# Zhongxu-Wang/ArtSpeech

Measured on AMD Instinct MI355X. Metric: mel frames/sec (whole job; per-GPU = value / n_gpus), acoustic-model inference path, batch 32 x 200-frame utterances, higher is better.
Workload: dtype f32 (f16x3 split-operand MFMA, fp32 accumulate)

## Files before the change

artspeech_amd/csrc/conv_gemm_h3.hip:

```cpp
#include "conv_gemm.h"
#include <cstring>
#include <type_traits>

typedef __attribute__((address_space(3))) void lds_void;

template <int I, int N, typename F>
static __device__ __forceinline__ void h3_for(F&& f)
{
    if constexpr (I < N) {
        f(std::integral_constant<int, I>{});
        h3_for<I + 1, N>(f);
    }
}

template <int WM, int WN, int WK, int KT, int NS, int NP, int TM = 2>
struct H3Cfg {
    static constexpr int QP = NP == 1 ? 2 : 4;
    static constexpr int BM = 32 * TM * WM, BN = 64 * WN;
    static constexpr int KBS = WK * KT;
    static constexpr int A_BLK = QP * BM * 16, B_BLK = QP * BN * 16;
    static constexpr int A_ST = KBS * A_BLK;
    static constexpr int STAGE = KBS * (A_BLK + B_BLK);
    static constexpr int RED = (WK - 1) * WM * WN * 32 * TM * 64 * 4;
    static constexpr int LDS = NS * STAGE > RED ? NS * STAGE : RED;
    static constexpr int NT = 64 * WM * WN * WK;
    static constexpr int ACH = KBS * QP * BM / NT;
    static constexpr int BCH = KBS * QP * BN / NT;
    static constexpr int NMF = 2 * TM * NP;
    static constexpr int NFR = (TM + 2) * (NP == 1 ? 1 : 2);
};

static constexpr int H3_OCC = 1;
static __device__ __forceinline__ int h3_problem_of(const H3Multi& mm)
{
    int pi = 0;
#pragma unroll
    for (int i = 1; i < H3_MAXP; ++i) pi += (i < mm.n && (int)blockIdx.x >= mm.p[i].wg0) ? 1 : 0;
    return pi;
}

template <int WM, int WN, int WK, int KT, int NS, int NP, int TM = 2>
static __device__ __forceinline__ void h3_tile(const H3Prob& prob, unsigned char* smem)
{
    using C = H3Cfg<WM, WN, WK, KT, NS, NP, TM>;
    static_assert(NS >= 2 && NS <= 4, "stages");
    constexpr int BM = C::BM, BN = C::BN, ACH = C::ACH, BCH = C::BCH, NT = C::NT, QP = C::QP, KBS = C::KBS;
    static_assert(NT == 256 && ACH * NT == KBS * QP * BM && BCH * NT == KBS * QP * BN && ACH >= 1 && BCH >= 1, "tile shape");

    const int tid = threadIdx.x, lane = tid & 63;
    const int wave = __builtin_amdgcn_readfirstlane(tid >> 6);
    const int wk = wave / (WM * WN), wmn = wave % (WM * WN), wm = wmn % WM, wn = wmn / WM;
    const int l31 = lane & 31, lk = lane >> 5;
    const ConvGemmArgs& a = prob.a;
    const H3Taps& tp = prob.tp;
    const int S = prob.S;
    const int tiles_m = (a.M + BM - 1) / BM;
    int lt, slice, tile, m0, n0, grp = 0, n_end = prob.col1;
    if (a.n_valid && S == 1) {
        const int nv = __builtin_amdgcn_readfirstlane(*a.n_valid);
        const int G = a.n_groups > 1 ? a.n_groups : 1;
        const int span = G > 1 ? a.group_cols : prob.col1 - prob.col0;
        const int ctv = (min(max(nv, 1), span) + BN - 1) / BN;
        const int tiles_v = tiles_m * G * ctv, per = (tiles_v + 7) >> 3;
        const int local = (int)blockIdx.x - prob.wg0;
        if ((local >> 3) >= per) return;
        lt = (local & 7) * per + (local >> 3);
        if (lt >= tiles_v) return;
        slice = 0;
        tile = lt;
        m0 = (lt % tiles_m) * BM;
        const int q = lt / tiles_m, tn = q / G;
        grp = q - tn * G;
        const int base = G > 1 ? grp * a.group_cols : prob.col0;
        n0 = base + tn * BN;
        n_end = min(G > 1 ? min(a.N, (grp + 1) * a.group_cols) : prob.col1, base + nv);
    } else {
        lt = logical_of((int)blockIdx.x - prob.wg0, prob.wgs);
        if (lt >= prob.tiles * S) return;
        slice = lt / prob.tiles;
        tile = lt - slice * prob.tiles;
        m0 = (tile % tiles_m) * BM;
        n0 = prob.col0 + (tile / tiles_m) * BN;
        if (a.n_groups > 1) {
            const int tpg = (a.group_cols + BN - 1) / BN, tn = tile / tiles_m;
            grp = tn / tpg;
            n0 = grp * a.group_cols + (tn - grp * tpg) * BN;
            n_end = min(a.N, (grp + 1) * a.group_cols);
        }
        if (a.n_valid) {
            n_end = min(n_end, (a.n_groups > 1 ? grp * a.group_cols : 0) + __builtin_amdgcn_readfirstlane(*a.n_valid));
            if (n0 >= n_end && n0 > 0) return;
        }
    }
    const int KB = a.Kp >> 4, KBx = (KB + 3) & ~3;
    const int NX = (a.src_col ? a.N_in : a.N) + 1;

    const int KB2 = (a.K2 + 15) >> 4, KBx2 = (KB2 + 3) & ~3;
    const unsigned w_bytes = ((unsigned)a.T * KBx + KBx2) * 4u * a.M * 16u;
    const __amdgpu_buffer_rsrc_t rsW = __builtin_amdgcn_make_buffer_rsrc(
        const_cast<unsigned char*>(reinterpret_cast<const unsigned char*>(a.Wh) + (size_t)grp * w_bytes), 0, (int)w_bytes, 0x00020000);
    const __amdgpu_buffer_rsrc_t rsX = __builtin_amdgcn_make_buffer_rsrc(
        const_cast<uint16_t*>(a.Xh), 0, (int)((unsigned)KBx * 4u * NX * 16u), 0x00020000);
    const __amdgpu_buffer_rsrc_t rsX2 = __builtin_amdgcn_make_buffer_rsrc(
        const_cast<uint16_t*>(KB2 ? a.Xh2 : a.Xh), 0, (int)((unsigned)KBx2 * 4u * NX * 16u), 0x00020000);

    (void)rsW;
    (void)rsX;
    (void)rsX2;
    unsigned a_voff[ACH];
#pragma unroll
    for (int i = 0; i < ACH; ++i) {
        const int c = tid + NT * i, kblk = c / (QP * BM), rem = c % (QP * BM), pk = rem / BM, row = rem % BM;
        a_voff[i] = (m0 + row) < a.M ? (unsigned)(((kblk * 4 + pk) * a.M + m0 + row) * 16) : OOB;
    }
    unsigned b_plane[BCH];
#pragma unroll
    for (int i = 0; i < BCH; ++i) {
        const int c = tid + NT * i, kblk = c / (QP * BN), pk = (c % (QP * BN)) / BN;
        b_plane[i] = (unsigned)((kblk * 4 + pk) * NX) * 16u;
    }
    const int j = n0 + tid % BN;
    unsigned tapmask = 0;
    int Wj = 0;
    if (j < n_end) {
        if (a.meta) {
            const unsigned long long md = a.meta[j];
            const int h = AS_META_h(md), w = AS_META_w(md);
            const int H = AS_META_H(md);
            Wj = AS_META_W(md);
            for (int t = 0; t < a.T; ++t) {
                const int byte = (int)(h3_tap_word(tp, t) >> ((t & 7) * 8)) & 0xff;
                const int dh = tp.wide ? 0 : (byte >> 4) - 8, dw = tp.wide ? byte - 128 : (byte & 15) - 8;
                if ((unsigned)(h + dh) < (unsigned)H && (unsigned)(w + dw) < (unsigned)Wj) tapmask |= 1u << t;
            }
        } else {
            tapmask = 0xffffffffu;
        }
    }
    const int jsrc = a.src_col ? (j < n_end ? a.src_col[j] : 0) : j;
    const int tA = tp.wide ? 16 : Wj, tC = jsrc + (tp.wide ? -128 : -8 * Wj - 8);

    const int it_per_tap = (KB + KBS - 1) / KBS;
    const int nit_all = a.T * it_per_tap + (KB2 + KBS - 1) / KBS;
    const int it_lo = (int)((long)nit_all * slice / S);
    const int n_it = (int)((long)nit_all * (slice + 1) / S) - it_lo;

    int s_t = min(it_lo / it_per_tap, a.T), s_kb = (it_lo - s_t * it_per_tap) * KBS;
    int kb_lim = s_t < a.T ? KB : KB2;
    __amdgpu_buffer_rsrc_t rsXc = s_t < a.T ? rsX : rsX2;
    const int a_step = KBS * 4 * a.M * 16, b_step = KBS * 4 * NX * 16;
    int a_soff = (s_t * KBx + s_kb) * 4 * a.M * 16, b_soff = s_kb * 4 * NX * 16;
    unsigned bv[BCH];
    auto set_tap = [&](int t) {
        int byte = (int)(h3_tap_word(tp, t) >> ((t & 7) * 8)) & 0xff;
        unsigned ok = 0u - ((tapmask >> (t & 31)) & 1u);
        if (t >= a.T) {
            byte = tp.wide ? 128 : 0x88;
            ok = 0u - (unsigned)(j < n_end);
        }
        const unsigned src = ((unsigned)((byte >> 4) * tA + (byte & 15) + tC) & ok) | ((unsigned)(NX - 1) & ~ok);
#pragma unroll
        for (int i = 0; i < BCH; ++i) bv[i] = b_plane[i] + src * 16u;
    };
    set_tap(s_t);
    auto advance = [&]() {
        s_kb += KBS;
        a_soff += a_step;
        b_soff += b_step;
        if (s_kb >= kb_lim) {
            if (s_t + 1 < a.T || (s_t + 1 == a.T && KB2 > 0)) {
                s_t += 1;
                s_kb = 0;
                a_soff = s_t * KBx * 4 * a.M * 16;
                b_soff = 0;
                if (s_t == a.T) {
                    kb_lim = KB2;
                    rsXc = rsX2;
                }
                set_tap(s_t);
            } else {
                s_kb -= KBS;
                a_soff -= a_step;
                b_soff -= b_step;
            }
        }
    };
    auto dma_a = [&](auto i_, int stage) {
#if __HIP_DEVICE_COMPILE__
        constexpr int i = decltype(i_)::value;
        __builtin_amdgcn_raw_ptr_buffer_load_lds(rsW, (lds_void*)(smem + stage * C::STAGE + wave * 1024 + i * (NT * 16)), 16, a_voff[i],
                                                 a_soff, 0, 0);
#endif
    };
    auto dma_b = [&](auto i_, int stage) {
#if __HIP_DEVICE_COMPILE__
        constexpr int i = decltype(i_)::value;
        __builtin_amdgcn_raw_ptr_buffer_load_lds(rsXc, (lds_void*)(smem + stage * C::STAGE + C::A_ST + wave * 1024 + i * (NT * 16)), 16, bv[i],
                                                 b_soff, 0, 0);
#endif
    };
    (void)bv;
    (void)a_soff;
    (void)b_soff;
    (void)rsXc;
    f16x8 fa[2][TM][2], fb[2][2][2];
    const int a_frag = (wk * KT * QP + lk) * BM * 16 + (wm * 32 * TM + l31) * 16;
    const int b_frag = C::A_ST + (wk * KT * QP + lk) * BN * 16 + (wn * 64 + l31) * 16;
    auto read_frag = [&](auto q_, auto set_, auto s_, int stage) {
        constexpr int q = decltype(q_)::value, set = decltype(set_)::value, s = decltype(s_)::value;
        constexpr int sec = q < TM ? 0 : (q < TM + 2 ? 1 : (q < 2 * TM + 2 ? 2 : 3));
        constexpr int i = sec == 0 ? q : (sec == 1 ? q - TM : (sec == 2 ? q - TM - 2 : q - 2 * TM - 2));
        constexpr int ab = sec == 0 || sec == 2 ? 0 : 1;
        constexpr int p = NP == 1 ? 0 : (sec == 0 || sec == 3 ? 0 : 1);
        const unsigned char* st = smem + stage * C::STAGE;
        if constexpr (ab == 0) fa[set][i][p] = *reinterpret_cast<const f16x8*>(st + a_frag + (s * QP + p * 2) * BM * 16 + i * 32 * 16);
        else fb[set][i][p] = *reinterpret_cast<const f16x8*>(st + b_frag + (s * QP + p * 2) * BN * 16 + i * 32 * 16);
    };
    f32x16 acc[TM][2];
#pragma unroll
    for (int i = 0; i < TM; ++i)
#pragma unroll
        for (int jn = 0; jn < 2; ++jn)
#pragma unroll
            for (int e = 0; e < 16; ++e) acc[i][jn][e] = 0.f;

    using I0 = std::integral_constant<int, 0>;
    constexpr int L = KT == 1 ? NS : NS - 1;
    static_assert(L >= 2, "KT > 1 needs three stages");
    for (int st = 0; st < L; ++st) {
        h3_for<0, ACH>([&](auto i_) { dma_a(i_, st); });
        h3_for<0, BCH>([&](auto i_) { dma_b(i_, st); });
        advance();
    }
    __syncthreads();
    h3_for<0, C::NFR>([&](auto q_) { read_frag(q_, I0{}, I0{}, 0); });
    __syncthreads();

    constexpr int NMI = KT * C::NMF;
    constexpr int M_ADV = ACH + BCH, NMS = M_ADV + 1;
    constexpr int SLOT0 = 0;
    auto stage_micro = [&](auto m_, auto p_) {
        constexpr int Mi = decltype(m_)::value, P = (decltype(p_)::value + L) % NS;
        if constexpr (Mi < ACH) dma_a(std::integral_constant<int, Mi>{}, P);
        else if constexpr (Mi < M_ADV) dma_b(std::integral_constant<int, Mi - ACH>{}, P);
        else advance();
    };
    auto slot_of_stage = [](int m) constexpr { return SLOT0 + (m * (NMI - SLOT0)) / NMS; };
    auto slot_of_frag = [](int s, int q) constexpr {
        return s * C::NMF + (q * (C::NMF - 2)) / C::NFR + (C::NMF > 4 ? 1 : 0);
    };
    auto step = [&](auto n_, auto s_, auto p_, auto f_) {
        constexpr int Nn = decltype(n_)::value, Ss = decltype(s_)::value, P = decltype(p_)::value, F = decltype(f_)::value;
        constexpr int grp_ = Nn / (2 * TM), i = (Nn % (2 * TM)) / 2, jn = Nn % 2;
        constexpr int PA = NP == 1 ? 0 : (grp_ == 1 ? 1 : 0);
        constexpr int PB = NP == 1 ? 0 : (grp_ == 0 ? 1 : 0);
        acc[i][jn] = __builtin_amdgcn_mfma_f32_32x32x16_f16(fa[F][i][PA], fb[F][jn][PB], acc[i][jn], 0, 0, 0);
        constexpr int slot = Ss * C::NMF + Nn;
        h3_for<0, NMS>([&](auto m_) {
            if constexpr (slot_of_stage(decltype(m_)::value) == slot) stage_micro(m_, p_);
        });
        h3_for<0, C::NFR>([&](auto q_) {
            if constexpr (slot_of_frag(Ss, decltype(q_)::value) == slot) {
                if constexpr (Ss + 1 < KT) read_frag(q_, std::integral_constant<int, F ^ 1>{}, std::integral_constant<int, Ss + 1>{}, P);
                else read_frag(q_, std::integral_constant<int, F ^ 1>{}, I0{}, (P + 1) % NS);
            }
        });
        __builtin_amdgcn_sched_barrier(0);
    };
    constexpr int PEND = (L - 2) * (ACH + BCH);
#define H3_ITER(U)                                                                                                \
    {                                                                                                             \
        h3_for<0, KT>([&](auto s_) {                                                                              \
            h3_for<0, C::NMF>([&](auto n_) {                                                                      \
                step(n_, s_, std::integral_constant<int, (U) % NS>{},                                             \
                     std::integral_constant<int, ((U) * KT + decltype(s_)::value) % 2>{});                        \
            });                                                                                                   \
        });                                                                                                       \
        asm volatile("s_waitcnt vmcnt(%0) lgkmcnt(0)\n\ts_barrier" ::"n"(PEND) : "memory");                     \
    }
    constexpr int PERIOD = (KT % 2 == 0) ? NS : (NS % 2 == 0 ? NS : 2 * NS);
    int it = 0;
    for (; it + PERIOD <= n_it; it += PERIOD) {
        h3_for<0, PERIOD>([&](auto u_) { H3_ITER(decltype(u_)::value) });
    }
    h3_for<0, PERIOD - 1>([&](auto u_) {
        if (it + decltype(u_)::value < n_it) H3_ITER(decltype(u_)::value)
    });
#undef H3_ITER
    asm volatile("s_waitcnt vmcnt(0)\n\ts_barrier" ::: "memory");

    if (WK > 1) {
        f32x4* red = reinterpret_cast<f32x4*>(smem);
        if (wk > 0) {
#pragma unroll
            for (int i = 0; i < TM; ++i)
#pragma unroll
                for (int jn = 0; jn < 2; ++jn)
#pragma unroll
                    for (int e4 = 0; e4 < 4; ++e4) {
                        f32x4 v = {acc[i][jn][4 * e4], acc[i][jn][4 * e4 + 1], acc[i][jn][4 * e4 + 2], acc[i][jn][4 * e4 + 3]};
                        red[((((wk - 1) * (WM * WN) + wmn) * 2 * TM + i * 2 + jn) * 4 + e4) * 64 + lane] = v;
                    }
        }
        __syncthreads();
        if (wk == 0)
#pragma unroll
            for (int s = 1; s < WK; ++s)
#pragma unroll
                for (int i = 0; i < TM; ++i)
#pragma unroll
                    for (int jn = 0; jn < 2; ++jn)
#pragma unroll
                        for (int e4 = 0; e4 < 4; ++e4) {
                            const f32x4 v = red[((((s - 1) * (WM * WN) + wmn) * 2 * TM + i * 2 + jn) * 4 + e4) * 64 + lane];
#pragma unroll
                            for (int c = 0; c < 4; ++c) acc[i][jn][4 * e4 + c] += v[c];
                        }
    }
    epilogue<TM, 2>(a, acc, m0, n0, wm, wn, l31, lk, S, slice, wk == 0, grp, n_end);
}

template <int WM, int WN, int WK, int KT, int NS, int NP, int TM = 2>
__global__ void __launch_bounds__(64 * WM * WN * WK, H3_OCC)
conv_gemm_h3_kernel(const H3Multi mm)
{
    extern __shared__ __attribute__((aligned(16))) unsigned char smem[];
    h3_tile<WM, WN, WK, KT, NS, NP, TM>(mm.p[h3_problem_of(mm)], smem);
}

template <int WM, int WN, int WK, int KT, int NS, int NP, int TM = 2>
static int launch_h3(const ConvGemmArgs* const* a, const int* S, int n, hipStream_t stream)
{
    using C = H3Cfg<WM, WN, WK, KT, NS, NP, TM>;
    AS_LDS_OPT_IN((&conv_gemm_h3_kernel<WM, WN, WK, KT, NS, NP, TM>), C::LDS);
    H3Multi mm;
    memset(&mm, 0, sizeof(mm));
    mm.n = n;
    int wg = 0;
    for (int i = 0; i < n; ++i) {
        H3Prob& p = mm.p[i];
        p.a = *a[i];
        if (h3_pack_taps(p.a, &p.tp) != AS_OK) return AS_EINVAL;
        const int tiles_n = p.a.n_groups > 1 ? p.a.n_groups * as_cdiv(p.a.group_cols, C::BN) : as_cdiv(p.a.N, C::BN);
        p.tiles = as_cdiv(p.a.M, C::BM) * tiles_n;
        p.col0 = 0;
        p.col1 = p.a.N;
        p.S = S[i];
        p.wg0 = wg;
        p.wgs = (p.tiles * p.S + 7) & ~7;
        wg += p.wgs;
    }
    hipLaunchKernelGGL((conv_gemm_h3_kernel<WM, WN, WK, KT, NS, NP, TM>), dim3(wg), dim3(C::NT), C::LDS, stream, mm);
    AS_CHECK_LAUNCH();
    return AS_OK;
}

template <int WM, int WN, int WK>
static int launch_h3_tile(const ConvGemmArgs* const* a, const int* S, int n, hipStream_t stream)
{
    if (a[0]->n_prod == 1) return launch_h3<WM, WN, WK, 1, 3, 1>(a, S, n, stream);
    return launch_h3<WM, WN, WK, 1, 3, 3>(a, S, n, stream);
}

int as_conv_gemm_h3_launch(const ConvGemmArgs* const* a, const int* S, int n, int choice, hipStream_t stream)
{
    if (n < 1 || n > H3_MAXP) return AS_EINVAL;
    for (int i = 0; i < n; ++i) {
        if (a[i]->n_prod != a[0]->n_prod || S[i] < 1) return AS_EINVAL;
        if ((double)as_kbx(a[i]->K) * 4.0 * ((a[i]->src_col ? a[i]->N_in : a[i]->N) + 1.0) * 16.0 >= 2147483648.0) return AS_EINVAL;
    }
    switch (choice) {
    case 2:
        if (a[0]->n_prod == 1) return AS_EINVAL;
        return launch_h3<1, 2, 2, 1, 2, 3, 1>(a, S, n, stream);
    case 22: return launch_h3_tile<2, 2, 1>(a, S, n, stream);
    case 21: return launch_h3_tile<2, 1, 2>(a, S, n, stream);
    case 12: return launch_h3_tile<1, 2, 2>(a, S, n, stream);
    case 14:
        if (a[0]->n_prod == 1) return launch_h3_tile<1, 2, 2>(a, S, n, stream);
        return launch_h3<1, 4, 1, 1, 3, 3>(a, S, n, stream);
    case 11: return launch_h3_tile<1, 1, 4>(a, S, n, stream);
    default: return AS_EINVAL;
    }
}

__global__ void __launch_bounds__(256)
split_f16x2_kernel(const float* __restrict__ x, int ldx, int K, int N, const int* __restrict__ n_valid, int lrelu, float slope,
                   u32x4_t* __restrict__ xh)
{
    const int wcol = (blockIdx.x * 256 + (threadIdx.x & ~63)) * 4;
    const int col = wcol + (threadIdx.x & 63);
    const int g = blockIdx.y;
    if (wcol > N) return;
    const int nv = n_valid ? min(max(*n_valid, 0), N) : N;
    if (wcol >= nv && wcol + 255 < N) return;
    const __amdgpu_buffer_rsrc_t rs = __builtin_amdgcn_make_buffer_rsrc(const_cast<float*>(x), 0, (int)(((unsigned)(K - 1) * ldx + N) * 4u), 0x00020000);
    float v[8][4];
#pragma unroll
    for (int r = 0; r < 8; ++r) {
        const int k = g * 8 + r;
#pragma unroll
        for (int c = 0; c < 4; ++c) v[r][c] = buf_load1(rs, (k < K && col + 64 * c < nv) ? (unsigned)(k * ldx + col + 64 * c) * 4u : OOB, 0);
    }
    const size_t NX = (size_t)N + 1;
    const size_t base = ((size_t)(g >> 1) * 4 + (g & 1)) * NX + col;
#pragma unroll
    for (int c = 0; c < 4; ++c) {
        if (col + 64 * c > N) break;
        if (col + 64 * c >= nv && col + 64 * c < N) continue;
        float t[8];
#pragma unroll
        for (int r = 0; r < 8; ++r) {
            float e = v[r][c];
            if (lrelu) e = e > 0.f ? e : slope * e;
            t[r] = e;
        }
        u32x4_t h, l;
        split2(t, h, l);
        xh[base + 64 * c] = h;
        xh[base + 64 * c + 2 * NX] = l;
    }
}

extern "C" size_t as_split_f16x2_bytes(int K, int N)
{
    if (K <= 0 || N <= 0) return 0;
    return (size_t)as_kbx(K) * 4 * ((size_t)N + 1) * 16;
}

int as_split_f16x2_launch(const float* x, int ldx, int K, int N, int lrelu, float slope, uint16_t* xh, hipStream_t stream,
                          const int32_t* n_valid)
{
    if ((double)K * ldx * 4.0 >= 2147483648.0) return AS_EINVAL;
    hipLaunchKernelGGL(split_f16x2_kernel, dim3(as_cdiv(N + 1, 1024), 2 * as_kbx(K)), dim3(256), 0, stream, x, ldx, K, N, n_valid, lrelu, slope,
                       reinterpret_cast<u32x4_t*>(xh));
    AS_CHECK_LAUNCH();
    return AS_OK;
}

extern "C" int as_split_f16x2_f32(const float* x, int ldx, int K, int N, int in_act, float in_slope, uint16_t* xh, as_stream_t stream)
{
    return as_split_f16x2_cap_f32(x, ldx, K, N, nullptr, in_act, in_slope, xh, stream);
}

extern "C" int as_split_f16x2_cap_f32(const float* x, int ldx, int K, int N, const int32_t* n_valid, int in_act, float in_slope, uint16_t* xh,
                                      as_stream_t stream)
{
    if (!x || !xh || K <= 0 || N < 0 || ldx < N || (in_act != 0 && in_act != 2) || !(fabsf(in_slope) <= 3.0e38f)) return AS_EINVAL;
    if ((reinterpret_cast<uintptr_t>(xh) & 15) != 0) return AS_EINVAL;
    if (N == 0) return AS_OK;
    AsProfScope prof__(AS_CLS_OTHER, 0, 8.0 * K * (double)N, (hipStream_t)stream);
    return as_split_f16x2_launch(x, ldx, K, N, in_act == 2, in_slope, xh, (hipStream_t)stream, n_valid);
}

extern "C" size_t as_prep_weight_f16x2_sc_bytes(int G, int Cout, int Cin, int T, int Cin2)
{
    if (G <= 0 || Cout <= 0 || Cin <= 0 || T <= 0 || Cin2 < 0) return 0;
    return (size_t)G * ((size_t)T * as_kbx(Cin) + (Cin2 ? as_kbx(Cin2) : 0)) * 4 * (size_t)Cout * 16;
}
extern "C" size_t as_prep_weight_f16x2_bytes(int G, int Cout, int Cin, int T) { return as_prep_weight_f16x2_sc_bytes(G, Cout, Cin, T, 0); }

extern "C" int as_prep_weight_f16x2_sc_host(const float* w, const float* w2, int G, int Cout, int Cin, int T, int Cin2, uint16_t* wh,
                                            float* scale_out)
{
    if (!w || !wh || !scale_out || G <= 0 || Cout <= 0 || Cin <= 0 || T <= 0 || Cin2 < 0 || ((Cin2 > 0) != (w2 != nullptr))) return AS_EINVAL;
    const size_t n = (size_t)G * Cout * Cin * T, n2 = (size_t)G * Cout * Cin2;
    float mx = 0.f;
    for (size_t i = 0; i < n + n2; ++i) {
        const float x = i < n ? w[i] : w2[i - n];
        const float v = x < 0 ? -x : x;
        if (!(v <= 3.0e38f)) return AS_EINVAL;
        mx = v > mx ? v : mx;
    }
    int e = 0;
    float scale = 1.0f;
    if (mx > 0.f) {
        frexpf(mx, &e);
        scale = ldexpf(1.0f, 14 - e);
    }
    const int KBx = as_kbx(Cin), KBx2 = Cin2 ? as_kbx(Cin2) : 0;
    const size_t blocks = (size_t)T * KBx + KBx2;
    const size_t total = as_prep_weight_f16x2_sc_bytes(G, Cout, Cin, T, Cin2) / 2;
    for (size_t i = 0; i < total; ++i) wh[i] = 0;
    auto put = [&](size_t block, int k, int m, float x) {
        const _Float16 h = (_Float16)x;
        const _Float16 l = (_Float16)(x - (float)h);
        const int kh = (k >> 3) & 1, e8 = k & 7;
        const size_t base = block * 4 * (size_t)Cout * 8;
        uint16_t hb, lb;
        __builtin_memcpy(&hb, &h, 2);
        __builtin_memcpy(&lb, &l, 2);
        wh[base + ((size_t)(0 * 2 + kh) * Cout + m) * 8 + e8] = hb;
        wh[base + ((size_t)(1 * 2 + kh) * Cout + m) * 8 + e8] = lb;
    };
    for (int g = 0; g < G; ++g)
        for (int m = 0; m < Cout; ++m) {
            for (int k = 0; k < Cin; ++k)
                for (int t = 0; t < T; ++t) put((size_t)g * blocks + (size_t)t * KBx + (k >> 4), k, m, w[(((size_t)g * Cout + m) * Cin + k) * T + t] * scale);
            for (int k = 0; k < Cin2; ++k) put((size_t)g * blocks + (size_t)T * KBx + (k >> 4), k, m, w2[((size_t)g * Cout + m) * Cin2 + k] * scale);
        }
    *scale_out = scale;
    return AS_OK;
}
extern "C" int as_prep_weight_f16x2_host(const float* w, int G, int Cout, int Cin, int T, uint16_t* wh, float* scale_out)
{
    return as_prep_weight_f16x2_sc_host(w, nullptr, G, Cout, Cin, T, 0, wh, scale_out);
}

static __device__ __forceinline__ float h3_wave_sum(float v)
{
#pragma unroll
    for (int o = 32; o > 0; o >>= 1) v += __shfl_xor(v, o);
    return v;
}

template <bool UP>
__global__ void __launch_bounds__(256)
adain_image_kernel(const AsAdainArgs a)
{
    const int lane = threadIdx.x & 63, wave = __builtin_amdgcn_readfirstlane(threadIdx.x >> 6);
    const int kb = blockIdx.x * 2 + (wave >> 1), kh = wave & 1, u = blockIdx.y;
    const int C = a.C;
    if (kb >= as_kbx(C)) return;
    const size_t NX = (size_t)a.N + 1;
    u32x4_t* xs = reinterpret_cast<u32x4_t*>(a.yh);
    const size_t plane = ((size_t)kb * 4 + kh) * NX;
    if (u == 0 && lane == 0) {
        xs[plane + a.N] = u32x4_t{0u, 0u, 0u, 0u};
        xs[plane + 2 * NX + a.N] = u32x4_t{0u, 0u, 0u, 0u};
    }
    const int o0 = a.col_off[u], L = a.col_w ? a.col_w[u] : a.col_off[u + 1] - o0;
    if (L <= 0) return;
    const int s0 = a.src_off ? a.src_off[u] : o0;
    const size_t gbase = a.gb_off ? (size_t)a.gb_off[u] : (size_t)u * a.ldgb;
    const int c0 = kb * 16 + kh * 8;
    float g1[8], bt[8], w0[8], w1[8], w2[8], pb[8];
#pragma unroll
    for (int r = 0; r < 8; ++r) {
        const int c = c0 + r < C ? c0 + r : C - 1;
        g1[r] = 1.0f + a.gb[gbase + (size_t)c * a.gb_sc];
        bt[r] = a.gb[gbase + (size_t)(C + c) * a.gb_sc];
        if (UP) { w0[r] = a.pool_w[c * 3 + 0]; w1[r] = a.pool_w[c * 3 + 1]; w2[r] = a.pool_w[c * 3 + 2]; pb[r] = a.pool_b[c]; }
    }
    const float* xr0 = a.x + s0;
    const size_t at0 = plane + (UP ? 2 * (size_t)o0 : (size_t)o0);
    float mean[8], rstd[8];
    auto resident = [&](auto rv_) {
        constexpr int RV = decltype(rv_)::value;
        float v[8][RV];
#pragma unroll
        for (int r = 0; r < 8; ++r) {
            const float* xr = xr0 + (size_t)(c0 + r < C ? c0 + r : C - 1) * a.ldx;
#pragma unroll
            for (int j = 0; j < RV; ++j) v[r][j] = xr[min(lane + 64 * j, L - 1)];
        }
#pragma unroll
        for (int r = 0; r < 8; ++r) {
            float sacc = 0.f;
#pragma unroll
            for (int j = 0; j < RV; ++j)
                if (lane + 64 * j < L) sacc += v[r][j];
            mean[r] = h3_wave_sum(sacc) / (float)L;
        }
#pragma unroll
        for (int r = 0; r < 8; ++r) {
            float vacc = 0.f;
#pragma unroll
            for (int j = 0; j < RV; ++j)
                if (lane + 64 * j < L) { const float d = __fsub_rn(v[r][j], mean[r]); vacc = __fmaf_rn(d, d, vacc); }
            rstd[r] = 1.0f / sqrtf(h3_wave_sum(vacc) / (float)L + 1e-5f);
        }
        if (UP && a.x_up) {
#pragma unroll
            for (int r = 0; r < 8; ++r) {
                if (c0 + r >= C) continue;
                float* ur = a.x_up + (size_t)(c0 + r) * a.ld_up + 2 * o0;
#pragma unroll
                for (int j = 0; j < RV; ++j) {
                    const int i = lane + 64 * j;
                    if (i < L) { ur[2 * i] = v[r][j]; ur[2 * i + 1] = v[r][j]; }
                }
            }
        }
#pragma unroll
        for (int r = 0; r < 8; ++r)
#pragma unroll
            for (int j = 0; j < RV; ++j)
                v[r][j] = (c0 + r < C && lane + 64 * j < L) ? as_adain_val(v[r][j], mean[r], rstd[r], g1[r], bt[r], a.lrelu) : 0.f;
#pragma unroll
        for (int j = 0; j < RV; ++j) {
            const int i = lane + 64 * j;
            if (64 * j >= L) break;
            if (!UP) {
                float t[8];
#pragma unroll
                for (int r = 0; r < 8; ++r) t[r] = v[r][j];
                u32x4_t h, l;
                split2(t, h, l);
                if (i < L) {
                    xs[at0 + i] = h;
                    xs[at0 + i + 2 * NX] = l;
                }
            } else {
                float e0[8], e1[8];
#pragma unroll
                for (int r = 0; r < 8; ++r) {
                    const float dn = __shfl_down(v[r][j], 1);
                    const float wr = j + 1 < RV ? __shfl(v[r][j + 1 < RV ? j + 1 : j], 0) : 0.f;
                    const float an = i + 1 < L ? (lane == 63 ? wr : dn) : 0.f;
                    float o0v, o1v;
                    as_convt_pair(v[r][j], an, w0[r], w1[r], w2[r], pb[r], &o0v, &o1v);
                    e0[r] = c0 + r < C ? o0v : 0.f;
                    e1[r] = c0 + r < C ? o1v : 0.f;
                }
                u32x4_t h, l, h2, l2;
                split2(e0, h, l);
                split2(e1, h2, l2);
                if (i < L) {
                    xs[at0 + 2 * i] = h;
                    xs[at0 + 2 * i + 2 * NX] = l;
                    xs[at0 + 2 * i + 1] = h2;
                    xs[at0 + 2 * i + 1 + 2 * NX] = l2;
                }
            }
        }
    };
    if (L <= 256) { resident(std::integral_constant<int, 4>{}); return; }
    if (L <= 512) { resident(std::integral_constant<int, 8>{}); return; }
    {
        size_t rowoff[8];
#pragma unroll
        for (int r = 0; r < 8; ++r) rowoff[r] = (size_t)(c0 + r < C ? c0 + r : C - 1) * a.ldx;
        float acc[8];
#pragma unroll
        for (int r = 0; r < 8; ++r) acc[r] = 0.f;
        int i = lane;
        for (; i + 192 < L; i += 256) {
            float t[4][8];
#pragma unroll
            for (int q = 0; q < 4; ++q)
#pragma unroll
                for (int r = 0; r < 8; ++r) t[q][r] = xr0[rowoff[r] + i + 64 * q];
#pragma unroll
            for (int q = 0; q < 4; ++q)
#pragma unroll
                for (int r = 0; r < 8; ++r) acc[r] += t[q][r];
        }
        for (; i < L; i += 64)
#pragma unroll
            for (int r = 0; r < 8; ++r) acc[r] += xr0[rowoff[r] + i];
#pragma unroll
        for (int r = 0; r < 8; ++r) { mean[r] = h3_wave_sum(acc[r]) / (float)L; acc[r] = 0.f; }
        i = lane;
        for (; i + 192 < L; i += 256) {
            float t[4][8];
#pragma unroll
            for (int q = 0; q < 4; ++q)
#pragma unroll
                for (int r = 0; r < 8; ++r) t[q][r] = xr0[rowoff[r] + i + 64 * q];
#pragma unroll
            for (int q = 0; q < 4; ++q)
#pragma unroll
                for (int r = 0; r < 8; ++r) { const float d = __fsub_rn(t[q][r], mean[r]); acc[r] = __fmaf_rn(d, d, acc[r]); }
        }
        for (; i < L; i += 64)
#pragma unroll
            for (int r = 0; r < 8; ++r) { const float d = __fsub_rn(xr0[rowoff[r] + i], mean[r]); acc[r] = __fmaf_rn(d, d, acc[r]); }
#pragma unroll
        for (int r = 0; r < 8; ++r) rstd[r] = 1.0f / sqrtf(h3_wave_sum(acc[r]) / (float)L + 1e-5f);
    }
    for (int i0 = lane; i0 < L; i0 += 128) {
        float xi[2][8], xn[2][8];
#pragma unroll
        for (int q = 0; q < 2; ++q) {
            const int i = min(i0 + 64 * q, L - 1);
#pragma unroll
            for (int r = 0; r < 8; ++r) {
                const float* xr = xr0 + (size_t)(c0 + r < C ? c0 + r : C - 1) * a.ldx;
                xi[q][r] = xr[i];
                if (UP) xn[q][r] = xr[min(i + 1, L - 1)];
            }
        }
#pragma unroll
        for (int q = 0; q < 2; ++q) {
            const int i = i0 + 64 * q;
            if (i >= L) break;
            float a0[8], a1[8];
#pragma unroll
            for (int r = 0; r < 8; ++r) {
                const bool ok = c0 + r < C;
                a0[r] = ok ? as_adain_val(xi[q][r], mean[r], rstd[r], g1[r], bt[r], a.lrelu) : 0.f;
                a1[r] = (UP && ok && i + 1 < L) ? as_adain_val(xn[q][r], mean[r], rstd[r], g1[r], bt[r], a.lrelu) : 0.f;
                if (UP && a.x_up && ok) {
                    float* ur = a.x_up + (size_t)(c0 + r) * a.ld_up + 2 * o0 + 2 * i;
                    ur[0] = xi[q][r];
                    ur[1] = xi[q][r];
                }
            }
            u32x4_t h, l;
            if (!UP) {
                split2(a0, h, l);
                xs[at0 + i] = h;
                xs[at0 + i + 2 * NX] = l;
            } else {
                float e0[8], e1[8];
#pragma unroll
                for (int r = 0; r < 8; ++r) {
                    as_convt_pair(a0[r], a1[r], w0[r], w1[r], w2[r], pb[r], &e0[r], &e1[r]);
                    if (c0 + r >= C) { e0[r] = 0.f; e1[r] = 0.f; }
                }
                split2(e0, h, l);
                xs[at0 + 2 * i] = h;
                xs[at0 + 2 * i + 2 * NX] = l;
                split2(e1, h, l);
                xs[at0 + 2 * i + 1] = h;
                xs[at0 + 2 * i + 1 + 2 * NX] = l;
            }
        }
    }
}

extern "C" int as_adain_image_f32(const AsAdainArgs* args_host, as_stream_t stream)
{
    if (!args_host) return AS_EINVAL;
    const AsAdainArgs& a = *args_host;
    if (!a.x || !a.gb || !a.col_off || !a.yh || a.C <= 0 || a.U <= 0 || a.N < 0 || a.gb_sc <= 0 || (!a.gb_off && a.ldgb <= 0)) return AS_EINVAL;
    if ((a.pool_w == nullptr) != (a.pool_b == nullptr) || (a.x_up && !a.pool_w)) return AS_EINVAL;
    if ((reinterpret_cast<uintptr_t>(a.yh) & 15) != 0) return AS_EINVAL;
    if (a.N == 0) return AS_OK;
    AsProfScope prof__(AS_CLS_ADAIN, 0, 8.0 * a.C * (double)a.N, (hipStream_t)stream);
    if (a.pool_w) hipLaunchKernelGGL(adain_image_kernel<true>, dim3(as_kbx(a.C) / 2, a.U), dim3(256), 0, (hipStream_t)stream, a);
    else hipLaunchKernelGGL(adain_image_kernel<false>, dim3(as_kbx(a.C) / 2, a.U), dim3(256), 0, (hipStream_t)stream, a);
    AS_CHECK_LAUNCH();
    return AS_OK;
}

extern "C" int as_adain_split_f32(const float* x, int ldx, int C, const float* gamma_beta, int ldgb, const int32_t* col_off, int B,
                                  int N, int lrelu, uint16_t* xs, as_stream_t stream)
{
    if (!x || !gamma_beta || !col_off || !xs || C <= 0 || B <= 0 || N < 0 || ldgb < 2 * C) return AS_EINVAL;
    AsAdainArgs a = {};
    a.x = x; a.ldx = ldx; a.C = C; a.gb = gamma_beta; a.ldgb = ldgb; a.gb_sc = 1; a.col_off = col_off; a.U = B; a.N = N; a.lrelu = lrelu; a.yh = xs;
    return as_adain_image_f32(&a, stream);
}

__global__ void __launch_bounds__(256)
rows_image_kernel(const float* __restrict__ x, int ldx, int K, int B, u32x4_t* __restrict__ xh)
{
    const int i = blockIdx.x * 256 + threadIdx.x;
    const int groups = 2 * as_kbx(K);
    if (i >= groups * (B + 1)) return;
    const int g = i / (B + 1), b = i % (B + 1);
    float t[8];
#pragma unroll
    for (int r = 0; r < 8; ++r) t[r] = (b < B && g * 8 + r < K) ? x[(size_t)b * ldx + g * 8 + r] : 0.f;
    u32x4_t h, l;
    split2(t, h, l);
    const size_t at = ((size_t)(g >> 1) * 4 + (g & 1)) * (B + 1) + b;
    xh[at] = h;
    xh[at + 2 * (size_t)(B + 1)] = l;
}

extern "C" int as_rows_image_f32(const float* x, int ldx, int K, int B, uint16_t* xh, as_stream_t stream)
{
    if (!x || !xh || K <= 0 || B <= 0 || ldx < K || (reinterpret_cast<uintptr_t>(xh) & 15) != 0) return AS_EINVAL;
    AsProfScope prof__(AS_CLS_OTHER, 0, 8.0 * K * (double)B, (hipStream_t)stream);
    hipLaunchKernelGGL(rows_image_kernel, dim3(as_cdiv((long)2 * as_kbx(K) * (B + 1), 256)), dim3(256), 0, (hipStream_t)stream, x, ldx, K, B,
                       reinterpret_cast<u32x4_t*>(xh));
    AS_CHECK_LAUNCH();
    return AS_OK;
}

#define LNS_COLS 32
#define LNS_PARTS 32
#define LNS_MAXG 4
__global__ void __launch_bounds__(1024)
channel_ln_split_kernel(const float* __restrict__ x, int ldx, int C, int N, const float* __restrict__ gamma1,
                        const float* __restrict__ beta1, const float* __restrict__ gamma2, const float* __restrict__ beta2, int n_split,
                        float eps, int relu, u32x4_t* __restrict__ xs, int KBx)
{
    __shared__ float red[LNS_PARTS][LNS_COLS + 1];
    const int col = threadIdx.x % LNS_COLS, part = threadIdx.x / LNS_COLS;
    const int j = blockIdx.x * LNS_COLS + col;
    const bool ok = j < N;
    const int grp = gamma2 ? j / n_split : 0;
    const float* gamma = gamma1 + (ptrdiff_t)grp * (gamma2 - gamma1);
    const float* beta = beta1 + (ptrdiff_t)grp * (beta2 - beta1);
    const int ngroups = 2 * KBx;
    float v[LNS_MAXG][8];
    float s = 0.f;
#pragma unroll
    for (int i = 0; i < LNS_MAXG; ++i)
#pragma unroll
        for (int r = 0; r < 8; ++r) {
            const int c = 8 * (part + i * LNS_PARTS) + r;
            v[i][r] = (ok && c < C) ? x[(size_t)c * ldx + j] : 0.f;
            s += v[i][r];
        }
    red[part][col] = s;
    __syncthreads();
    float tot = 0.f;
#pragma unroll
    for (int q = 0; q < LNS_PARTS; ++q) tot += red[q][col];
    const float mean = tot / (float)C;
    __syncthreads();
    float q2 = 0.f;
#pragma unroll
    for (int i = 0; i < LNS_MAXG; ++i)
#pragma unroll
        for (int r = 0; r < 8; ++r) {
            const int c = 8 * (part + i * LNS_PARTS) + r;
            const float d = __fsub_rn(v[i][r], mean);
            if (c < C) q2 = __fmaf_rn(d, d, q2);
        }
    red[part][col] = q2;
    __syncthreads();
    tot = 0.f;
#pragma unroll
    for (int q = 0; q < LNS_PARTS; ++q) tot += red[q][col];
    const float rs = 1.0f / sqrtf(tot / (float)C + eps);
    const size_t NX = (size_t)N + 1;
    if (blockIdx.x == 0 && col == 0) {
#pragma unroll
        for (int i = 0; i < LNS_MAXG; ++i) {
            const int g = part + i * LNS_PARTS;
            if (g < ngroups)
                for (int p = 0; p < 2; ++p) xs[((size_t)(g >> 1) * 4 + (g & 1) + 2 * p) * NX + N] = u32x4_t{0u, 0u, 0u, 0u};
        }
    }
    if (!ok) return;
#pragma unroll
    for (int i = 0; i < LNS_MAXG; ++i) {
        const int g = part + i * LNS_PARTS;
        if (g >= ngroups) continue;
        float t[8];
#pragma unroll
        for (int r = 0; r < 8; ++r) {
            const int c = 8 * g + r;
            float o = 0.f;
            if (c < C) {
                o = __fmaf_rn(__fmul_rn(__fsub_rn(v[i][r], mean), rs), gamma[c], beta[c]);
                if (relu) o = o < 0.f ? 0.f : o;
            }
            t[r] = o;
        }
        u32x4_t h, l;
        split2(t, h, l);
        const size_t at = ((size_t)(g >> 1) * 4 + (g & 1)) * NX + j;
        xs[at] = h;
        xs[at + 2 * NX] = l;
    }
}

extern "C" int as_channel_layernorm_split_f32(const float* x, int ldx, int C, int N, const float* gamma, const float* beta,
                                              const float* gamma2, const float* beta2, int n_split, float eps, int relu, uint16_t* xs,
                                              as_stream_t stream)
{
    if (!x || !xs || !gamma || !beta || C <= 0 || C > 8 * LNS_PARTS * LNS_MAXG || N <= 0 || ldx < N ||
        ((gamma2 == nullptr) != (beta2 == nullptr)) || (gamma2 && n_split <= 0) || (reinterpret_cast<uintptr_t>(xs) & 15) != 0)
        return AS_EINVAL;
    const int KBx = as_kbx(C);
    AsProfScope prof__(AS_CLS_LN, 8.0 * C * N, 8.0 * C * (double)N, (hipStream_t)stream);
    hipLaunchKernelGGL(channel_ln_split_kernel, dim3(as_cdiv(N, LNS_COLS)), dim3(1024), 0, (hipStream_t)stream, x, ldx, C, N, gamma, beta,
                       gamma2, beta2, n_split, eps, relu, reinterpret_cast<u32x4_t*>(xs), KBx);
    AS_CHECK_LAUNCH();
    return AS_OK;
}
```

Baseline: 1.763 million.

## Use permlane/DPP wave reduction and scalar-load per-utterance metadata in AdaIN image kernel

Replaces the shfl_xor wave-sum with v_permlane32/16_swap plus DPP row operations, so reductions avoid LDS-backed bpermute. Per-utterance offsets and gamma/beta/pool weights are loaded through the constant address space with inline-asm SGPR hints, making them scalar loads. Row loads are issued before the gamma/beta loads, and the kernel is split into helpers. Wave-to-channel-group mapping is unchanged in substance. The inline asm depends on gfx950-specific permlane swap instructions.

```diff
diff --git a/artspeech_amd/csrc/conv_gemm_h3.hip b/artspeech_amd/csrc/conv_gemm_h3.hip
--- a/artspeech_amd/csrc/conv_gemm_h3.hip
+++ b/artspeech_amd/csrc/conv_gemm_h3.hip
@@ -507,126 +507,163 @@
     return as_prep_weight_f16x2_sc_host(w, nullptr, G, Cout, Cin, T, 0, wh, scale_out);
 }
 
+template <int CTRL>
+static __device__ __forceinline__ float h3_dpp(float v)
+{
+    return __builtin_bit_cast(float, __builtin_amdgcn_mov_dpp(__builtin_bit_cast(int, v), CTRL, 0xf, 0xf, true));
+}
 static __device__ __forceinline__ float h3_wave_sum(float v)
 {
-#pragma unroll
-    for (int o = 32; o > 0; o >>= 1) v += __shfl_xor(v, o);
+    float x0 = v, x1 = v;
+    asm("s_nop 1\n\tv_permlane32_swap_b32 %0, %1" : "+v"(x0), "+v"(x1));
+    v = x0 + x1;
+    x0 = v;
+    x1 = v;
+    asm("s_nop 1\n\tv_permlane16_swap_b32 %0, %1" : "+v"(x0), "+v"(x1));
+    v = x0 + x1;
+    v += h3_dpp<0x128>(v);
+    v += h3_dpp<0x124>(v);
+    v += h3_dpp<0x4E>(v);
+    v += h3_dpp<0xB1>(v);
     return v;
 }
 
-template <bool UP>
-__global__ void __launch_bounds__(256)
-adain_image_kernel(const AsAdainArgs a)
-{
-    const int lane = threadIdx.x & 63, wave = __builtin_amdgcn_readfirstlane(threadIdx.x >> 6);
-    const int kb = blockIdx.x * 2 + (wave >> 1), kh = wave & 1, u = blockIdx.y;
-    const int C = a.C;
-    if (kb >= as_kbx(C)) return;
-    const size_t NX = (size_t)a.N + 1;
-    u32x4_t* xs = reinterpret_cast<u32x4_t*>(a.yh);
-    const size_t plane = ((size_t)kb * 4 + kh) * NX;
-    if (u == 0 && lane == 0) {
-        xs[plane + a.N] = u32x4_t{0u, 0u, 0u, 0u};
-        xs[plane + 2 * NX + a.N] = u32x4_t{0u, 0u, 0u, 0u};
-    }
-    const int o0 = a.col_off[u], L = a.col_w ? a.col_w[u] : a.col_off[u + 1] - o0;
-    if (L <= 0) return;
-    const int s0 = a.src_off ? a.src_off[u] : o0;
-    const size_t gbase = a.gb_off ? (size_t)a.gb_off[u] : (size_t)u * a.ldgb;
-    const int c0 = kb * 16 + kh * 8;
-    float g1[8], bt[8], w0[8], w1[8], w2[8], pb[8];
+template <typename T>
+static __device__ __forceinline__ T h3_ldu(const T* p)
+{
+    return *(const __attribute__((address_space(4))) T*)p;
+}
+
+struct AdainLay {
+    int o0, L, s0;
+    size_t gbase;
+};
+static __device__ __forceinline__ AdainLay adain_lay(const AsAdainArgs& a, int u)
+{
+    const int32_t* pw = a.col_w ? a.col_w + u : a.col_off + u + 1;
+    const int32_t* ps = a.src_off ? a.src_off + u : a.col_off + u;
+    const int32_t* pg = a.gb_off ? a.gb_off + u : a.col_off + u;
+    asm volatile("" : "+s"(pw), "+s"(ps), "+s"(pg));
+    int o0 = h3_ldu(a.col_off + u), w = h3_ldu(pw), s = h3_ldu(ps), g = h3_ldu(pg);
+    asm volatile("" : "+s"(o0), "+s"(w), "+s"(s), "+s"(g));
+    AdainLay l;
+    l.o0 = o0;
+    l.L = a.col_w ? w : w - o0;
+    l.s0 = s;
+    l.gbase = a.gb_off ? (size_t)g : (size_t)u * a.ldgb;
+    return l;
+}
+
+static __device__ __forceinline__ void adain_gb(const float* gb, int gb_sc, int c0, int C, float (&gm)[8], float (&bt)[8])
+{
 #pragma unroll
     for (int r = 0; r < 8; ++r) {
         const int c = c0 + r < C ? c0 + r : C - 1;
-        g1[r] = 1.0f + a.gb[gbase + (size_t)c * a.gb_sc];
-        bt[r] = a.gb[gbase + (size_t)(C + c) * a.gb_sc];
-        if (UP) { w0[r] = a.pool_w[c * 3 + 0]; w1[r] = a.pool_w[c * 3 + 1]; w2[r] = a.pool_w[c * 3 + 2]; pb[r] = a.pool_b[c]; }
-    }
-    const float* xr0 = a.x + s0;
-    const size_t at0 = plane + (UP ? 2 * (size_t)o0 : (size_t)o0);
+        gm[r] = gb[(size_t)c * gb_sc];
+        bt[r] = gb[(size_t)(C + c) * gb_sc];
+    }
+}
+
+template <int RV>
+static __device__ __forceinline__ void adain_rows(float (&v)[8][RV], const float* xr0, int ldx, int c0, int C, int lane, int Lm1)
+{
+#pragma unroll
+    for (int r = 0; r < 8; ++r) {
+        const float* xr = xr0 + (size_t)(c0 + r < C ? c0 + r : C - 1) * ldx;
+#pragma unroll
+        for (int j = 0; j < RV; ++j) v[r][j] = xr[(unsigned)min(lane + 64 * j, Lm1)];
+    }
+}
+
+struct AdainUp { float w0[8], w1[8], w2[8], pb[8]; };
+
+template <bool UP, int RV>
+static __device__ __forceinline__ void adain_resident(const AsAdainArgs& a, float (&v)[8][RV], int lane, int L, int o0, int c0,
+                                                      const float (&gm)[8], const float (&bt)[8], const AdainUp& up, u32x4_t* xs, size_t at0,
+                                                      size_t NX)
+{
+    const int C = a.C;
     float mean[8], rstd[8];
-    auto resident = [&](auto rv_) {
-        constexpr int RV = decltype(rv_)::value;
-        float v[8][RV];
+#pragma unroll
+    for (int r = 0; r < 8; ++r) {
+        float sacc = 0.f;
+#pragma unroll
+        for (int j = 0; j < RV; ++j)
+            if (lane + 64 * j < L) sacc += v[r][j];
+        mean[r] = h3_wave_sum(sacc) / (float)L;
+    }
+#pragma unroll
+    for (int r = 0; r < 8; ++r) {
+        float vacc = 0.f;
+#pragma unroll
+        for (int j = 0; j < RV; ++j)
+            if (lane + 64 * j < L) { const float d = __fsub_rn(v[r][j], mean[r]); vacc = __fmaf_rn(d, d, vacc); }
+        rstd[r] = 1.0f / sqrtf(h3_wave_sum(vacc) / (float)L + 1e-5f);
+    }
+    if (UP && a.x_up) {
 #pragma unroll
         for (int r = 0; r < 8; ++r) {
-            const float* xr = xr0 + (size_t)(c0 + r < C ? c0 + r : C - 1) * a.ldx;
-#pragma unroll
-            for (int j = 0; j < RV; ++j) v[r][j] = xr[min(lane + 64 * j, L - 1)];
-        }
-#pragma unroll
-        for (int r = 0; r < 8; ++r) {
-            float sacc = 0.f;
-#pragma unroll
-            for (int j = 0; j < RV; ++j)
-                if (lane + 64 * j < L) sacc += v[r][j];
-            mean[r] = h3_wave_sum(sacc) / (float)L;
-        }
-#pragma unroll
-        for (int r = 0; r < 8; ++r) {
-            float vacc = 0.f;
-#pragma unroll
-            for (int j = 0; j < RV; ++j)
-                if (lane + 64 * j < L) { const float d = __fsub_rn(v[r][j], mean[r]); vacc = __fmaf_rn(d, d, vacc); }
-            rstd[r] = 1.0f / sqrtf(h3_wave_sum(vacc) / (float)L + 1e-5f);
-        }
-        if (UP && a.x_up) {
+            if (c0 + r >= C) continue;
+            float* ur = a.x_up + (size_t)(c0 + r) * a.ld_up + 2 * o0;
+#pragma unroll
+            for (int j = 0; j < RV; ++j) {
+                const int i = lane + 64 * j;
+                if (i < L) { ur[2 * i] = v[r][j]; ur[2 * i + 1] = v[r][j]; }
+            }
+        }
+    }
+#pragma unroll
+    for (int r = 0; r < 8; ++r) {
+        const float g1 = 1.0f + gm[r];
+#pragma unroll
+        for (int j = 0; j < RV; ++j)
+            v[r][j] = (c0 + r < C && lane + 64 * j < L) ? as_adain_val(v[r][j], mean[r], rstd[r], g1, bt[r], a.lrelu) : 0.f;
+    }
+#pragma unroll
+    for (int j = 0; j < RV; ++j) {
+        const int i = lane + 64 * j;
+        if (64 * j >= L) break;
+        if (!UP) {
+            float t[8];
+#pragma unroll
+            for (int r = 0; r < 8; ++r) t[r] = v[r][j];
+            u32x4_t h, l;
+            split2(t, h, l);
+            if (i < L) {
+                xs[at0 + i] = h;
+                xs[at0 + i + 2 * NX] = l;
+            }
+        } else {
+            float e0[8], e1[8];
 #pragma unroll
             for (int r = 0; r < 8; ++r) {
-                if (c0 + r >= C) continue;
-                float* ur = a.x_up + (size_t)(c0 + r) * a.ld_up + 2 * o0;
-#pragma unroll
-                for (int j = 0; j < RV; ++j) {
-                    const int i = lane + 64 * j;
-                    if (i < L) { ur[2 * i] = v[r][j]; ur[2 * i + 1] = v[r][j]; }
-                }
-            }
-        }
-#pragma unroll
-        for (int r = 0; r < 8; ++r)
-#pragma unroll
-            for (int j = 0; j < RV; ++j)
-                v[r][j] = (c0 + r < C && lane + 64 * j < L) ? as_adain_val(v[r][j], mean[r], rstd[r], g1[r], bt[r], a.lrelu) : 0.f;
-#pragma unroll
-        for (int j = 0; j < RV; ++j) {
-            const int i = lane + 64 * j;
-            if (64 * j >= L) break;
-            if (!UP) {
-                float t[8];
-#pragma unroll
-                for (int r = 0; r < 8; ++r) t[r] = v[r][j];
-                u32x4_t h, l;
-                split2(t, h, l);
-                if (i < L) {
-                    xs[at0 + i] = h;
-                    xs[at0 + i + 2 * NX] = l;
-                }
-            } else {
-                float e0[8], e1[8];
-#pragma unroll
-                for (int r = 0; r < 8; ++r) {
-                    const float dn = __shfl_down(v[r][j], 1);
-                    const float wr = j + 1 < RV ? __shfl(v[r][j + 1 < RV ? j + 1 : j], 0) : 0.f;
-                    const float an = i + 1 < L ? (lane == 63 ? wr : dn) : 0.f;
-                    float o0v, o1v;
-                    as_convt_pair(v[r][j], an, w0[r], w1[r], w2[r], pb[r], &o0v, &o1v);
-                    e0[r] = c0 + r < C ? o0v : 0.f;
-                    e1[r] = c0 + r < C ? o1v : 0.f;
-                }
-                u32x4_t h, l, h2, l2;
-                split2(e0, h, l);
-                split2(e1, h2, l2);
-                if (i < L) {
-                    xs[at0 + 2 * i] = h;
-                    xs[at0 + 2 * i + 2 * NX] = l;
-                    xs[at0 + 2 * i + 1] = h2;
-                    xs[at0 + 2 * i + 1 + 2 * NX] = l2;
-                }
-            }
-        }
-    };
-    if (L <= 256) { resident(std::integral_constant<int, 4>{}); return; }
-    if (L <= 512) { resident(std::integral_constant<int, 8>{}); return; }
+                const float dn = __shfl_down(v[r][j], 1);
+                const float wr = j + 1 < RV ? __shfl(v[r][j + 1 < RV ? j + 1 : j], 0) : 0.f;
+                const float an = i + 1 < L ? (lane == 63 ? wr : dn) : 0.f;
+                float o0v, o1v;
+                as_convt_pair(v[r][j], an, up.w0[r], up.w1[r], up.w2[r], up.pb[r], &o0v, &o1v);
+                e0[r] = c0 + r < C ? o0v : 0.f;
+                e1[r] = c0 + r < C ? o1v : 0.f;
+            }
+            u32x4_t h, l, h2, l2;
+            split2(e0, h, l);
+            split2(e1, h2, l2);
+            if (i < L) {
+                xs[at0 + 2 * i] = h;
+                xs[at0 + 2 * i + 2 * NX] = l;
+                xs[at0 + 2 * i + 1] = h2;
+                xs[at0 + 2 * i + 1 + 2 * NX] = l2;
+            }
+        }
+    }
+}
+
+template <bool UP>
+static __device__ __forceinline__ void adain_long(const AsAdainArgs& a, const float* xr0, int lane, int L, int o0, int c0, const float (&gm)[8],
+                                                  const float (&bt)[8], const AdainUp& up, u32x4_t* xs, size_t at0, size_t NX)
+{
+    const int C = a.C;
+    float mean[8], rstd[8];
     {
         size_t rowoff[8];
 #pragma unroll
@@ -669,6 +706,9 @@
 #pragma unroll
         for (int r = 0; r < 8; ++r) rstd[r] = 1.0f / sqrtf(h3_wave_sum(acc[r]) / (float)L + 1e-5f);
     }
+    float g1[8];
+#pragma unroll
+    for (int r = 0; r < 8; ++r) g1[r] = 1.0f + gm[r];
     for (int i0 = lane; i0 < L; i0 += 128) {
         float xi[2][8], xn[2][8];
 #pragma unroll
@@ -706,7 +746,7 @@
                 float e0[8], e1[8];
 #pragma unroll
                 for (int r = 0; r < 8; ++r) {
-                    as_convt_pair(a0[r], a1[r], w0[r], w1[r], w2[r], pb[r], &e0[r], &e1[r]);
+                    as_convt_pair(a0[r], a1[r], up.w0[r], up.w1[r], up.w2[r], up.pb[r], &e0[r], &e1[r]);
                     if (c0 + r >= C) { e0[r] = 0.f; e1[r] = 0.f; }
                 }
                 split2(e0, h, l);
@@ -718,6 +758,61 @@
             }
         }
     }
+}
+
+template <bool UP>
+static __device__ __forceinline__ void adain_item(const AsAdainArgs& a, int lane, int u, int g, const AdainLay& lay)
+{
+    const int C = a.C, L = lay.L, o0 = lay.o0;
+    const size_t NX = (size_t)a.N + 1;
+    u32x4_t* xs = reinterpret_cast<u32x4_t*>(a.yh);
+    const size_t plane = ((size_t)(g >> 1) * 4 + (g & 1)) * NX;
+    const int c0 = g * 8;
+    if (L > 0) {
+        const float* xr0 = a.x + lay.s0;
+        const size_t at0 = plane + (UP ? 2 * (size_t)o0 : (size_t)o0);
+        float gm[8], bt[8];
+        AdainUp up;
+        if (UP) {
+#pragma unroll
+            for (int r = 0; r < 8; ++r) {
+                const int c = c0 + r < C ? c0 + r : C - 1;
+                up.w0[r] = h3_ldu(a.pool_w + c * 3 + 0);
+                up.w1[r] = h3_ldu(a.pool_w + c * 3 + 1);
+                up.w2[r] = h3_ldu(a.pool_w + c * 3 + 2);
+                up.pb[r] = h3_ldu(a.pool_b + c);
+            }
+        }
+        if (L <= 256) {
+            float v[8][4];
+            adain_rows<4>(v, xr0, a.ldx, c0, C, lane, L - 1);
+            adain_gb(a.gb + lay.gbase, a.gb_sc, c0, C, gm, bt);
+            adain_resident<UP, 4>(a, v, lane, L, o0, c0, gm, bt, up, xs, at0, NX);
+        } else if (L <= 512) {
+            float v[8][8];
+            adain_rows<8>(v, xr0, a.ldx, c0, C, lane, L - 1);
+            adain_gb(a.gb + lay.gbase, a.gb_sc, c0, C, gm, bt);
+            adain_resident<UP, 8>(a, v, lane, L, o0, c0, gm, bt, up, xs, at0, NX);
+        } else {
+            adain_gb(a.gb + lay.gbase, a.gb_sc, c0, C, gm, bt);
+            adain_long<UP>(a, xr0, lane, L, o0, c0, gm, bt, up, xs, at0, NX);
+        }
+    }
+    if (u == 0 && lane == 0) {
+        xs[plane + a.N] = u32x4_t{0u, 0u, 0u, 0u};
+        xs[plane + 2 * NX + a.N] = u32x4_t{0u, 0u, 0u, 0u};
+    }
+}
+
+template <bool UP>
+__global__ void __launch_bounds__(256)
+adain_image_kernel(const AsAdainArgs a)
+{
+    const int lane = threadIdx.x & 63, wave = __builtin_amdgcn_readfirstlane(threadIdx.x >> 6);
+    const int g = blockIdx.x * 4 + wave, u = blockIdx.y;
+    if (g >= 2 * as_kbx(a.C)) return;
+    const AdainLay lay = adain_lay(a, u);
+    adain_item<UP>(a, lane, u, g, lay);
 }
 
 extern "C" int as_adain_image_f32(const AsAdainArgs* args_host, as_stream_t stream)
```

Result: no change. 1.763 million (median of 2 runs) (-0.0%).
